# LittleWat/multichannel-semseg-with-uda

Measured on AMD Instinct MI355X. Metric: RGB-D img/s (6x480x640) MCD train step, drn_d_38, higher is better.
Workload: dtype f32 (operands split 2-way into scaled fp16, 3 cross terms on the fp16 MFMA pipe, fp32 accumulate)

## Files before the change

include/mcdseg.h:

```cpp
#ifndef MCDSEG_H
#define MCDSEG_H

#include <stddef.h>
#include <stdint.h>

#ifdef __cplusplus
extern "C" {
#endif
#pragma GCC visibility push(default)

#define MCDSEG_VERSION 101

int mcdseg_version(void);
const char* mcdseg_last_error(void);

#define MCDSEG_COMM_ID_BYTES 128
int mcdseg_comm_unique_id(void* id128);
int mcdseg_comm_init(void** comm, int32_t nranks, const void* id128, int32_t rank);
int mcdseg_comm_destroy(void* comm);
int mcdseg_allreduce(float* buf, int64_t count, void* comm, void* stream);

int32_t mcdseg_option_count(void);
const char* mcdseg_option_name(int32_t index);
int mcdseg_set_option(const char* name, int64_t value);
// ... 18 lines not shown
int mcdseg_conv_dgrad(const mcdseg_conv_desc* d, const float* dy, const float* wp_dgrad, float* dx, void* stream);
#define MCDSEG_MATH_F16X3 3
#define MCDSEG_MATH_BF16X6 6
#define MCDSEG_MATH_F16X1 1
int mcdseg_conv_split_packed_bytes(const mcdseg_conv_desc* d, int32_t math, int64_t* fprop_bytes, int64_t* dgrad_bytes);
int32_t mcdseg_conv_split_direct_ok(const mcdseg_conv_desc* d);
int64_t mcdseg_conv_split_stat_rows(const mcdseg_conv_desc* d);
int64_t mcdseg_conv_split_stat_rows_for(const mcdseg_conv_desc* d, int32_t math, int32_t presplit);
int32_t mcdseg_conv_split_window_ok(const mcdseg_conv_desc* d, int32_t math, int32_t presplit, int32_t dgrad);
int32_t mcdseg_conv_split_tile_config(int32_t M, int64_t P, int32_t presplit);
int mcdseg_absmax(const float* x, int64_t n, float* bound, void* stream);
int mcdseg_conv_split_pack_weights(const mcdseg_conv_desc* d, int32_t math, const float* w, void* wp_fprop, void* wp_dgrad,
                                   float* w_bound, void* stream);
int mcdseg_conv_split_pack_weights_multi(const int64_t* ptrs, const int32_t* dims, int32_t n, int32_t math, float* bounds,
                                         void* stream);
int mcdseg_conv_split_fprop(const mcdseg_conv_desc* d, int32_t math, const float* x, const void* x_cb, const float* x_bound,
                            const void* wp_fprop, const float* w_bound, const float* bias, float* y, float* stat_partials,
                            void* stream);
int mcdseg_conv_split_fprop_affine(const mcdseg_conv_desc* d, int32_t math, const float* x, const void* x_cb, const float* x_bound,
                                   const void* wp_fprop, const float* w_bound, const float* scale, const float* shift,
                                   const float* residual, int32_t relu, float* y, void* stream);
int mcdseg_conv_split_dgrad(const mcdseg_conv_desc* d, int32_t math, const float* dy, const void* dy_cb, const float* dy_bound,
                            const void* wp_dgrad, const float* w_bound, float* dx, void* stream);
int mcdseg_conv_split_dgrad_add(const mcdseg_conv_desc* d, int32_t math, const float* dy, const void* dy_cb, const float* dy_bound,
                                const void* wp_dgrad, const float* w_bound, const float* addend, float* dx, int32_t part, void* stream);
int64_t mcdseg_conv_split_parts(const mcdseg_conv_desc* d, int32_t math, int32_t presplit, int32_t dgrad);
int32_t mcdseg_conv_split_rest_pingpong(const mcdseg_conv_desc* d, int32_t math, int32_t presplit, int32_t dgrad);
int32_t mcdseg_conv_split_wide_pingpong(const mcdseg_conv_desc* d, int32_t math, int32_t presplit, int32_t dgrad);
int mcdseg_conv_split_fprop_part(const mcdseg_conv_desc* d, int32_t math, const float* x, const void* x_cb, const float* x_bound,
                                 const void* wp_fprop, const float* w_bound, const float* bias, float* y, float* stat_partials,
// ... 238 lines not shown
```

multichannel-semseg-with-uda_amd/csrc/conv_gemm_split.hip:

```cpp
#include <cstdlib>
#include <type_traits>

#include "conv_split_params.h"
#include "options.h"

namespace {


template <class P, int WM, int WN, int WAVES_M, int WAVES_N, bool DGRAD, bool PRESPLIT>
__global__ __launch_bounds__(256, 2) void conv_gemm_split_kernel(ConvSplitParams p) {
  constexpr int BM = 32 * WM * WAVES_M;
  constexpr int BN = 32 * WN * WAVES_N;
  constexpr int NT = 256;
  static_assert(WAVES_M * WAVES_N == 4, "4 waves per workgroup");
  constexpr int B_ITEMS = BN * 2 / NT;
  constexpr int NP = P::NP;
  constexpr int NQ = 2 * NP;
  typedef typename P::frag frag;
  constexpr int A_CHUNKS = NQ * BM;
  constexpr int A_ITERS = (A_CHUNKS + NT - 1) / NT;
  constexpr bool A_EXACT = (A_CHUNKS % NT) == 0;
  constexpr bool A_DMA = A_EXACT;
  constexpr int A_ITERS_DMA = ((2 * P::NPU * BM) % NT == 0) ? (2 * P::NPU * BM) / NT : A_ITERS;
  constexpr int A_BYTES = NQ * BM * 16, B_BYTES = NQ * BN * 16;
// ... 755 lines not shown
    for (int u = t; u < T * 2 * MT; u += 256) {
      const int mm = u % MT, r = u / MT;
      const int h = r & 1, tap = r >> 1;
      float v[8];
#pragma unroll
      for (int el = 0; el < 8; ++el) v[el] = tile[mm * row_len + (8 * h + el) * T + tap];
      typename P::frag q[NP];
      split_frag<P>(v, inv_scale, q);
      const int64_t base = ((int64_t)chunk * T + tap) * (2 * NP) * (int64_t)Mp * 8;
#pragma unroll
      for (int pc = 0; pc < NP; ++pc) *reinterpret_cast<typename P::frag*>(out + base + ((pc * 2 + h) * (int64_t)Mp + m0 + mm) * 8) = q[pc];
    }
  }
}

int split_check(const mcdseg_conv_desc* d, int math, const char* who, bool operands = true) {
  MCD_REQUIRE(d != nullptr, "%s: null descriptor", who);
  MCD_REQUIRE(mcd_math_known(math), "%s: math must be MCDSEG_MATH_BF16X6, MCDSEG_MATH_F16X3 or MCDSEG_MATH_F16X1 (got %d)", who, math);
  MCD_REQUIRE(d->N > 0 && d->Cin > 0 && d->H > 0 && d->W > 0 && d->Cout > 0, "%s: non-positive dims", who);
  MCD_REQUIRE(d->KH > 0 && d->KW > 0 && d->stride > 0 && d->dil > 0 && d->pad >= 0, "%s: bad kernel geometry", who);
  const int ho = (d->H + 2 * d->pad - d->dil * (d->KH - 1) - 1) / d->stride + 1;
  const int wo = (d->W + 2 * d->pad - d->dil * (d->KW - 1) - 1) / d->stride + 1;
  MCD_REQUIRE(ho == d->Ho && wo == d->Wo, "%s: Ho/Wo (%d,%d) do not match geometry (%d,%d)", who, d->Ho, d->Wo, ho, wo);
  MCD_REQUIRE(!operands || ((int64_t)d->N * d->Cin * d->H * d->W * 4 < (1ll << 31) && (int64_t)d->N * d->Cout * d->Ho * d->Wo * 4 < (1ll << 31)),
              "%s: activation tensor must stay below 2 GiB (32-bit buffer offsets); split the batch", who);
  return 0;
}

int64_t split_image_bytes(int math, int M, int K, int T) {
  return (int64_t)(round_up(K, 16) / 16) * T * 2 * mcd_math_pieces(math) * mcd_mp(M) * 16;
// ... 206 lines not shown
  math = mcd_storage_math(math);
  MCD_REQUIRE(ptrs && dims && n > 0 && n <= 32767, "conv_split_pack_weights_multi: bad table");
  MCD_REQUIRE(math == MCDSEG_MATH_BF16X6 || math == MCDSEG_MATH_F16X3, "conv_split_pack_weights_multi: unknown math %d", math);
  MCD_REQUIRE(math != MCDSEG_MATH_F16X3 || bounds != nullptr, "conv_split_pack_weights_multi: f16x3 needs the bounds array");
  hipStream_t st = (hipStream_t)stream;
  const unsigned pack_blocks = (unsigned)(mcd_opt(MCD_OPT_PACK_BLOCKS) > 0 ? mcd_opt(MCD_OPT_PACK_BLOCKS) : 192);
  if (math == MCDSEG_MATH_F16X3) {
    (void)hipMemsetAsync(bounds, 0, sizeof(float) * (size_t)n, st);
    hipLaunchKernelGGL(absmax_multi_kernel, dim3(48, (unsigned)n), dim3(256), 0, st, ptrs, dims);
    MCD_LAUNCH_CHECK("absmax_multi");
    hipLaunchKernelGGL(pack_weights_multi_kernel<SplitF16x3>, dim3(pack_blocks, 2u * (unsigned)n), dim3(256), 0, st, ptrs, dims);
  } else {
    hipLaunchKernelGGL(pack_weights_multi_kernel<SplitBf16x6>, dim3(pack_blocks, 2u * (unsigned)n), dim3(256), 0, st, ptrs, dims);
  }
  MCD_LAUNCH_CHECK("conv_split_pack_weights_multi");
  return 0;
}

static int split_cb_bytes(const mcdseg_conv_desc* d, int math, int C, int HW, const void* cb, int* piece_bytes, long long* piece_stride) {
  *piece_bytes = 0;
  *piece_stride = 0;
  if (cb == nullptr) return 0;
  MCD_REQUIRE((C % 8) == 0, "conv_split: a pre-split operand needs a channel count divisible by 8 (got %d)", C);
  MCD_REQUIRE(d->Ncb == 0 || d->Ncb >= d->N, "conv_split: Ncb (%d) must be 0 or at least N (%d)", d->Ncb, d->N);
  const int64_t b = (int64_t)d->N * C * HW * 2;
  MCD_REQUIRE(b < (1ll << 31), "conv_split: one piece of the pre-split operand exceeds 2 GiB; split the batch");
  *piece_bytes = (int)b;
  *piece_stride = math == MCDSEG_MATH_F16X1 ? 0 : (long long)(d->Ncb ? d->Ncb : d->N) * C * HW * 2;
  return 0;
}
// ... 218 lines not shown
```

multichannel-semseg-with-uda_amd/csrc/options.h:

```cpp
#pragma once
#include <stdint.h>

#define MCD_OPTIONS(X)                                                                                                       \
  X(BN_STATS_ONE, 1024)                     \
  X(BN_REVERSE, 1)                              \
  X(BN_V4, 1)                                         \
  X(BIGTILE_MIN_SLOTS, 1024)                               \
  X(WIDETILE_MIN_SLOTS, 1024)                                                                 \
  X(DGRAD_INTERLEAVE, 1)       \
  X(DGRAD_ADD_LDS, 1)                   \
  X(PACK_BLOCKS, 192)                               \
  X(PP_MIN_ROUNDS, 2)          \
  X(PP_CUS, 0)                 \
  X(PINGPONG, 3)               \
  X(PP_WIDE_FILL, 80)                               \
  X(PP_WIDE128, 1)                                                                                \
  X(PP_DEEP, 1)                \
  X(SKIP_DEAD_TAPS, 1)         \
  X(THIN_WINDOW, 1)                                                           \
  X(WGRAD_WGS, 1024)                                  \
  X(WGRAD_THIN_TR, 1)                                                               \
  X(WGRAD_TR64, 1)                                                    \
  X(WGRAD_BIG, 1)                                                                       \
  X(WGRAD_PP_CUS, 0)                          \
  X(WGRAD_PP, 2)                                          \
  X(WGRAD_PP3, 1)                                                                 \
// ... 13 lines not shown
```

multichannel-semseg-with-uda_amd/mcdseg/_lib.py:

```python
import ctypes
import glob
import os
import subprocess
import threading

HERE = os.path.dirname(os.path.abspath(__file__))
PKG = os.path.dirname(HERE)
REPO = os.path.dirname(PKG)
CSRC = os.path.join(PKG, "csrc")
INCLUDE = os.path.join(REPO, "include")
LIB_PATH = os.environ.get("MCDSEG_LIB") or os.path.join(HERE, "libmcdseg.so")

c_void_p, c_int, c_i32, c_i64, c_float, c_size_t = (ctypes.c_void_p, ctypes.c_int, ctypes.c_int32, ctypes.c_int64,
                                                    ctypes.c_float, ctypes.c_size_t)


class ConvDesc(ctypes.Structure):
    _fields_ = [(n, c_i32) for n in ("N", "Cin", "H", "W", "Cout", "KH", "KW", "stride", "pad", "dil", "Ho", "Wo", "Ncb")]


_P = ctypes.POINTER
_SIGNATURES = {
    "mcdseg_version": (c_int, []),
    "mcdseg_last_error": (ctypes.c_char_p, []),
# ... 26 lines not shown
    "mcdseg_up8_uncertain_loss_bwd": (c_int, [c_void_p] * 5 + [c_i64, c_void_p, c_void_p, c_float, c_void_p, c_float] + [c_void_p] * 4 +
                                      [c_i32] * 5 + [c_void_p]),
    "mcdseg_up8_std_sum": (c_int, [c_void_p] * 3 + [c_i32] * 5 + [c_void_p]),
    "mcdseg_dann_down_workspace_bytes": (c_size_t, [c_i32] * 5),
    "mcdseg_dann_down_fwd": (c_int, [c_void_p] * 6 + [c_i32] * 5 + [c_void_p]),
    "mcdseg_dann_down_bwd": (c_int, [c_void_p] * 11 + [c_i32] * 6 + [c_void_p, c_size_t, c_void_p]),
    "mcdseg_dann_tail_save_bytes": (c_size_t, [c_i32] * 2),
    "mcdseg_dann_tail_workspace_bytes": (c_size_t, [c_i32] * 2),
    "mcdseg_dann_tail_fwd": (c_int, [c_void_p] * 10 + [c_float, c_float, c_i32] + [c_void_p] * 3 + [c_i32] * 3 + [c_void_p]),
    "mcdseg_dann_tail_bwd": (c_int, [c_void_p] * 16 + [c_i32] * 4 + [c_void_p, c_size_t, c_void_p]),
    "mcdseg_depth_image_u8": (c_int, [c_void_p, c_void_p] + [c_i32] * 4 + [c_void_p]),
    "mcdseg_absmax": (c_int, [c_void_p, c_i64, c_void_p, c_void_p]),
    "mcdseg_conv_split_packed_bytes": (c_int, [_P(ConvDesc), c_i32, _P(c_i64), _P(c_i64)]),
    "mcdseg_conv_split_pack_weights": (c_int, [_P(ConvDesc), c_i32] + [c_void_p] * 5),
    "mcdseg_conv_split_pack_weights_multi": (c_int, [c_void_p, c_void_p, c_i32, c_i32, c_void_p, c_void_p]),
    "mcdseg_conv_split_fprop": (c_int, [_P(ConvDesc), c_i32] + [c_void_p] * 9),
    "mcdseg_conv_split_fprop_affine": (c_int, [_P(ConvDesc), c_i32] + [c_void_p] * 8 + [c_i32, c_void_p, c_void_p]),
    "mcdseg_conv_split_dgrad": (c_int, [_P(ConvDesc), c_i32] + [c_void_p] * 7),
    "mcdseg_conv_split_parts": (c_i64, [_P(ConvDesc), c_i32, c_i32, c_i32]),
    "mcdseg_conv_split_rest_pingpong": (c_i32, [_P(ConvDesc), c_i32, c_i32, c_i32]),
    "mcdseg_conv_split_wide_pingpong": (c_i32, [_P(ConvDesc), c_i32, c_i32, c_i32]),
    "mcdseg_conv_split_fprop_part": (c_int, [_P(ConvDesc), c_i32] + [c_void_p] * 8 + [c_i32, c_void_p]),
    "mcdseg_conv_split_dgrad_part": (c_int, [_P(ConvDesc), c_i32] + [c_void_p] * 6 + [c_i32, c_void_p]),
    "mcdseg_conv_split_dgrad_add": (c_int, [_P(ConvDesc), c_i32] + [c_void_p] * 7 + [c_i32, c_void_p]),
    "mcdseg_split_cb": (c_int, [c_void_p, c_void_p, c_void_p, c_i32, c_i32, c_i32, c_i32, c_void_p]),
    "mcdseg_split_cb_padded": (c_int, [c_void_p, c_void_p, c_void_p, c_i32, c_i32, c_i32, c_i32, c_void_p]),
    "mcdseg_unsplit_cb": (c_int, [c_void_p, c_void_p, c_i32, c_i32, c_i32, c_i32, c_void_p, c_void_p]),
    "mcdseg_stage_join": (c_int, [c_void_p] * 7 + [c_i32] * 4 + [c_void_p]),
    "mcdseg_bn_apply_cb": (c_int, [c_void_p] * 11 + [c_i32] * 5 + [c_void_p]),
    "mcdseg_bn_bwd_apply_cb": (c_int, [c_void_p] * 13 + [c_i32] * 6 + [c_void_p]),
# ... 394 lines not shown
```

multichannel-semseg-with-uda_amd/mcdseg/ops.py:

```python
import collections
import contextlib
import ctypes
import os
import threading
import types
import weakref

import torch

from . import _lib
from ._lib import ConvDesc, check, get_option, lib

WEIGHT_EPOCH = 0


def bump_weight_epoch(params=None):
    global WEIGHT_EPOCH
    if params is None:
        WEIGHT_EPOCH += 1
        return
    for p in params:
        p._mcd_epoch = getattr(p, "_mcd_epoch", 0) + 1


# ... 357 lines not shown
    members = []
    for pw in list(_PACK_REGISTRY):
        w = pw._weight() if pw._weight is not None else None
        if (w is None or pw._dims is None or pw._dims[4] != CONV_MATH or w.device != device or pw.wd is None or pw.wf is None
                or pw._dims[2] > 72):
            continue
        members.append((pw, w))
    if len(members) < 2:
        return
    members.sort(key=lambda m: m[1].data_ptr())
    sig = tuple((w.data_ptr(), pw.wf.data_ptr(), pw.wd.data_ptr()) + pw._dims for pw, w in members)
    tab = _PACK_TABLES.get((device, CONV_MATH))
    if tab is None or tab["sig"] != sig:
        n = len(members)
        bounds = torch.zeros(n, dtype=torch.float32, device=device)
        ptrs, dims = [], []
        for i, (pw, w) in enumerate(members):
            ptrs += [w.data_ptr(), pw.wf.data_ptr(), pw.wd.data_ptr(), bounds.data_ptr() + 4 * i]
            dims += [pw._dims[0], pw._dims[1], pw._dims[2], 0]
        tab = dict(sig=sig, bounds=bounds, ptrs=torch.tensor(ptrs, dtype=torch.int64).to(device),
                   dims=torch.tensor(dims, dtype=torch.int32).to(device))
        _PACK_TABLES[(device, CONV_MATH)] = tab
    if _scaled():
        for i, (pw, _) in enumerate(members):
            pw.w_bound = tab["bounds"][i:i + 1]
    n = len(members)
    nbytes = sum(4 * w.numel() + 2 * pw.wf.numel() + 2 * pw.wd.numel() for pw, w in members)
    with _timed("pack_weights_multi_kernel", (0, nbytes)):
        check(L.mcdseg_conv_split_pack_weights_multi(_p(tab["ptrs"]), _p(tab["dims"]), n, MATH_ID[CONV_MATH],
                                                     _p(tab["bounds"]) if _scaled() else None, _stream()), "conv_split_pack_weights_multi")
    for pw, w in members:
        if pw._dims[3]:
            d = ConvDesc(1, pw._dims[1], 8, 8, pw._dims[0], 7, 7, 1, 3, 1, 8, 8)
            check(L.mcdseg_conv_split_pack_weights(ctypes.byref(d), MATH_ID[CONV_MATH], _p(w.detach()), _p(pw.wf), None,
                                                   _p(pw.w_bound) if _scaled() else None, _stream()), "conv_split_pack_weights")
        pw.key = PackedWeights._key_of(w)


def _is_split(w_image):
    return w_image.dtype == torch.int16


MAX_CONV_BYTES = int(os.environ.get("MCDSEG_MAX_CONV_BYTES", str((1 << 31) - (1 << 26))))


# ... 218 lines not shown
    return _wgrad_name(d, _wgrad_variant(d, have_cb))


def _wgrad_thin_tr(desc):
    return _wgrad_variant(desc, True) == 15


def _wgrad_split_plan(desc, have_cb=False):
    return _wgrad_variant(desc, have_cb) >= 10


def _wgrad_reads_cb(desc):
    return _wgrad_variant(desc, True) >= 11 and desc.Cin % 8 == 0 and desc.Cout % 8 == 0


def _conv_wgrad(desc, x, dy, x_cb=None, dy_cb=None, x_bound=None, dy_bound=None):
    L, total = lib(), None
    if x_cb is None or dy_cb is None:
        x_cb = dy_cb = None
    pieces = _batch_pieces(desc, wgrad_cb=x_cb is not None)
    if x_cb is not None and len(pieces) > 1 and desc.Cin <= 16:
        x_cb = dy_cb = None
        pieces = _batch_pieces(desc, wgrad_cb=False)
    split = _wgrad_split_plan(desc, x_cb is not None)
    if split and x_cb is None:
        x_bound, dy_bound = _bound_or_measure(x, x_bound), _bound_or_measure(dy, dy_bound)
    for a, b, d in _launches(desc, pieces, x_cb is not None):
        ws = _ws(L.mcdseg_conv_wgrad_workspace_bytes(ctypes.byref(d)), (x if x is not None else x_cb).device)
        dw = torch.empty((desc.Cout, desc.Cin, desc.KH, desc.KW), dtype=torch.float32, device=ws.device)
        name = "" if LAUNCH_TIMER is None else (wgrad_split_kernel_name(d, x_cb is not None) if split else
                                                 wgrad_kernel_name(desc.Cout, desc.Cin, desc.KH * desc.KW))
        with _timed(name, conv_work(d)):
            if split:
                check(L.mcdseg_conv_split_wgrad(ctypes.byref(d), MATH_ID[CONV_MATH], _p(_sl(x, a, b)), _cb_slice(x_cb, a, desc.Cin, desc.H * desc.W),
                                                _p(x_bound), _p(_sl(dy, a, b)), _cb_slice(dy_cb, a, desc.Cout, desc.Ho * desc.Wo), _p(dy_bound),
                                                _p(dw), _p(ws), ctypes.c_size_t(ws.numel() * 4), _stream()), "conv_split_wgrad")
            else:
                check(L.mcdseg_conv_wgrad(ctypes.byref(d), _p(x[a:b]), _p(dy[a:b]), _p(dw), _p(ws), ctypes.c_size_t(ws.numel() * 4),
                                          _stream()), "conv_wgrad")
        _on_launch_stream(ws, dw)
        if total is None:
            total = dw
        else:
            with torch.cuda.stream(_LAUNCH.stream or torch.cuda.current_stream()):
                total.add_(dw)
    return total


OVERLAP_WGRAD = os.environ.get("MCDSEG_OVERLAP_WGRAD", "2")
if OVERLAP_WGRAD not in ("0", "1", "2"):
    raise ValueError("MCDSEG_OVERLAP_WGRAD must be 0, 1 or 2, got %r" % OVERLAP_WGRAD)
_SIDE = {}
_PENDING = {}


def _side_stream(device):
    key = device.index if device.index is not None else torch.cuda.current_device()
    if key not in _SIDE:
        _SIDE[key] = torch.cuda.Stream(device=device)
    return _SIDE[key]


def join_side_streams(device_index=None):
# ... 66 lines not shown
    if ev is not None:
        torch.cuda.current_stream().wait_event(ev)
        anchor._mcd_fwd_ev = None


def _fwd_sync_record(anchor):
    ev = torch.cuda.Event()
    ev.record(torch.cuda.current_stream())
    anchor._mcd_fwd_ev = ev


class _LateGrad(torch.autograd.Function):

    @staticmethod
    def forward(ctx, w):
        return w.view_as(w)

    @staticmethod
    def backward(ctx, g):
        join_side_streams(g.device.index)
        return g


class late_weight_grads:

    def __init__(self, root):
        self.root, self.mods = root, []

    def __enter__(self):
        if OVERLAP_WGRAD == "2" and torch.is_grad_enabled():
            for m in self.root.modules():
                if isinstance(getattr(m, "_packed", None), PackedWeights) and getattr(m, "_w_late", None) is None:
                    w = m.weight
                    if w.is_cuda and w.requires_grad and (not getattr(w, "_post_accumulate_grad_hooks", None) or
                                                          getattr(w, "_mcd_grad_sink", None) is not None):
# ... 44 lines not shown
def _conv_backward(desc, x, dy, wd, need_dx, need_dw, dy_cb=None, x_cb=None, dy_bound=None, x_bound=None, w_bound=None, defer=False, param=None,
                   dx_addend=None, dx16=False):
    mode = OVERLAP_WGRAD
    sink = getattr(param, "_mcd_grad_sink", None) if param is not None else None
    if mode == "2" and not (defer and x_cb is not None and dy_cb is not None):
        mode = "0"
    if mode != "0" and LAUNCH_TIMER is not None and LAUNCH_TIMER.wants("conv_wgrad"):
        mode = "0"
    if mode == "2" and not _room_to_defer(x.device):
        mode = "0"
        WGRAD_STREAM_STATS["no_room"] += 1
    if not (need_dx and need_dw and mode != "0"):
        if sink is not None and need_dw:
            sink(param, None)
        return ((_dgrad_any(desc, dy, wd, dy_cb, dy_bound, w_bound, dx_addend, dx16) if need_dx else None),
                (_conv_wgrad(desc, x, dy, x_cb, dy_cb, x_bound, dy_bound) if need_dw else None))
    main = torch.cuda.current_stream()
    side = _side_stream(x.device)
    key = side.device.index
    if _scaled() and dy is not None:
        dy_bound = _bound_or_measure(dy, dy_bound)
    side.wait_stream(main)
    _LAUNCH.stream, _LAUNCH.keep = side, [x, dy, x_cb, dy_cb, x_bound, dy_bound]
    try:
        dw = _conv_wgrad(desc, x, dy, x_cb, dy_cb, x_bound, dy_bound)
    finally:
        keep, _LAUNCH.stream, _LAUNCH.keep = _LAUNCH.keep, None, None
    dx = _dgrad_any(desc, dy, wd, dy_cb, dy_bound, w_bound, dx_addend, dx16)
    if mode == "1":
        main.wait_stream(side)
        if sink is not None:
            sink(param, None)
        return dx, dw
    if sink is not None:
        with torch.cuda.stream(side):
            sink(param, dw)
    WGRAD_STREAM_STATS["deferred"] += 1
    ev = torch.cuda.Event()
    ev.record(side)
    _PENDING[key] = (ev, main)
    held = _HELD.setdefault(key, collections.deque())
    held.append((ev, keep))
    while len(held) > MAX_LAG:
        main.wait_event(held.popleft()[0])
    torch.autograd.Variable._execution_engine.queue_callback(join_side_streams)
    return dx, dw


MASK_NONE = "none"
MASK_Y = "y"
MASK_Y_CB = "y_cb"
MASK_Z = "z"
MASK_BITS = "bits"


def _channel_reduce(dy, mask=MASK_NONE, src=None, z=None, mean=None, rstd=None, gamma=None, beta=None, want_bound=False, train=True):
    L = lib()
    n, c, hw = dy.shape[0], dy.shape[1], dy.shape[2] * dy.shape[3]
    ws = _ws(L.mcdseg_bn_bwd_workspace_bytes(n, c, hw), dy.device)
    dgamma = torch.empty(c, dtype=torch.float32, device=dy.device) if z is not None else None
    dbeta = torch.empty(c, dtype=torch.float32, device=dy.device)
    bound = torch.empty(1, dtype=torch.float32, device=dy.device) if want_bound else None
    tail = (int(train), n, c, hw, _p(ws), ctypes.c_size_t(ws.numel() * 4), _stream())
    if mask == MASK_BITS:
        with _timed("bn_bwd_reduce", (0, 4 * n * c * hw * 2)):
            check(L.mcdseg_bn_bwd_reduce_mask(_p(dy), _p(src), _p(z), _p(mean), _p(rstd), _p(gamma) if want_bound else None, _p(dgamma),
                                              _p(dbeta), _p(bound), *tail), "bn_bwd_reduce_mask")
    elif mask == MASK_Z:
        with _timed("bn_bwd_reduce", (0, 4 * n * c * hw * 2)):
            check(L.mcdseg_bn_bwd_reduce_zmask(_p(dy), _p(z), _p(mean), _p(rstd), _p(gamma), _p(beta), _p(dgamma), _p(dbeta), _p(bound),
                                               *tail), "bn_bwd_reduce_zmask")
    else:
        with _timed("bn_bwd_reduce", (0, 4 * n * c * hw * (1 + (mask == MASK_Y) + (z is not None)))):
            check(L.mcdseg_bn_bwd_reduce(_p(dy), _p(src) if mask == MASK_Y else None, _p(src) if mask == MASK_Y_CB else None,
                                         MATH_ID.get(CONV_MATH, 0), _p(z), _p(mean), _p(rstd), _p(dgamma), _p(dbeta),
                                         _p(gamma) if want_bound else None, _p(bound), int(train), n, c, hw, int(mask != MASK_NONE),
# ... 246 lines not shown
                                                  _p(dbeta), _p(dz_bound), mask, 1, n, c, hw, _p(ws), ctypes.c_size_t(ws.numel() * 4),
                                                  _stream()), "bn_bwd_reduce_half")
            dz_cb = torch.empty(elems, dtype=torch.int16, device=dy.device)
            if plan.has_res and need.residual:
                dres = torch.empty_like(dy) if plan.relu else dy
            p_dres = _p(dres) if plan.relu else None
            with _timed("bn_bwd_apply_half", (0, elems * (6 + (2 if mask == 4 else 0) + (2 if p_dres is not None else 0)))):
                check(L.mcdseg_bn_bwd_apply_half(_p(dy), src, _p(z), _p(ctx.z_bound), _p(mean), _p(rstd), _p(gamma), _p(beta), _p(dgamma),
                                                 _p(dbeta), _p(dz_cb), _p(dz_bound), p_dres, mask, 1, n, c, hw, _stream()),
                      "bn_bwd_apply_half")
        else:
            if plan.y_fp32:
                y, y_cb = materialize(y, y_cb, y_bound), None
            y_mask = (y if y_cb is None else None) if plan.relu else None
            src = {MASK_NONE: None, MASK_Y: y_mask, MASK_Y_CB: y_cb, MASK_BITS: ctx.rmask, MASK_Z: None if plan.use_cb else y_mask}[plan.mask]
            dgamma, dbeta, dz_bound = _channel_reduce(dy, plan.mask, src, z, mean, rstd, gamma, beta, plan.want_bound, plan.training)
            if plan.has_res and need.residual:
                dres = torch.empty_like(z) if plan.relu else dy
            if not plan.skip_dz:
                dz = torch.empty_like(z)
            dz_cb = _bn_bwd_apply(dy, plan.mask, src, plan.use_cb, z, mean, rstd, gamma, beta, dgamma, dbeta, dz, dres, dz_bound, plan.training)
            if plan.x_fp32_bwd:
                x = materialize(x, ctx.x_cb, ctx.x_bound)
            if DEBUG_TAPE is not None:
                DEBUG_TAPE.append(dict(dy=dy, dz=dz, dz_cb=dz_cb, dz_bound=dz_bound, dgamma=dgamma, dbeta=dbeta, dres=dres, shape=(n, c, hw),
                                       z=z, y=y_mask, mean=mean, rstd=rstd, gamma=gamma, beta=beta, zmask=plan.mask == MASK_Z))
            if dres is not None and plan.res_half:
                dres = pack_bf16_units(dres)
        if ctx.res_box is not None and dres is not None:
            other, last = ctx.res_box.arrive()
            if last:
                dres = dres if other is None else dres + other
            else:
                ctx.res_box.leave(dres if other is None else dres + other)
                dres = None
        addend, dx_last = ctx.in_box.arrive() if (ctx.in_box is not None and need.x) else (None, True)
        dx, dw = _conv_backward(desc, x, dz, ctx.wd, need.x, need.weight, dz_cb, x_cb, dz_bound, x_bound, ctx.w_bound, defer=ctx.defer_ok,
                                param=ctx.w_param, dx_addend=addend, dx16=ctx.x_half)
        if not dx_last:
            ctx.in_box.leave(dx)
            dx = None
        dbias = _channel_reduce(dz)[1] if (plan.has_bias and need.conv_bias) else None
        return tuple(_GroupGrads(x=dx, weight=dw, gamma=dgamma if need.gamma else None, beta=dbeta if need.beta else None, residual=dres,
                                 conv_bias=dbias))


def _conv_bn_act_inference(x, conv, bn, relu, residual):
    L = lib()
    x = _req(materialize(x), "conv input")
    residual = _req(materialize(residual) if residual is not None else None, "residual")
    desc = conv_desc(x.shape, conv.weight.shape, conv.stride[0], conv.padding[0], conv.dilation[0])
    wf, _, _ = conv._packed.get(conv.weight, desc)
    c = desc.Cout
    scale = torch.empty(c, dtype=torch.float32, device=x.device)
    shift = torch.empty(c, dtype=torch.float32, device=x.device)
    check(L.mcdseg_bn_eval_affine(_p(bn.weight), _p(bn.bias), _p(bn.running_mean), _p(bn.running_var), _p(conv.bias), c,
                                  float(bn.eps), _p(scale), _p(shift), _stream()), "bn_eval_affine")
# ... 1178 lines not shown
```

multichannel-semseg-with-uda_amd/mcdseg/optim.py:

```python
import os

import torch

from . import dist as mdist
from . import ops

_ALIGN = 64
DP_OVERLAP = os.environ.get("MCDSEG_DP_OVERLAP", "0") == "1"
DP_BUCKET_MB = float(os.environ.get("MCDSEG_DP_BUCKET_MB", "25"))


class _FlatOptimizer(torch.optim.Optimizer):
    _require_gpu = True
    _STATE = ()

    def __init__(self, params, defaults):
        super().__init__(params, defaults)
        self._flat = None

    @property
    def _name(self):
        return type(self).__name__

    def _all_params(self):
# ... 19 lines not shown
            offs.append(total)
            total += (p.numel() + _ALIGN - 1) // _ALIGN * _ALIGN
        fp = torch.zeros(total, dtype=torch.float32, device=dev)
        fs = [torch.zeros(total, dtype=torch.float32, device=dev) for _ in self._STATE]
        fg = torch.zeros(total, dtype=torch.float32, device=dev)
        views = {}
        for p, o in zip(params, offs):
            n = p.numel()
            pv = fp[o:o + n].view(p.shape)
            pv.copy_(p.data)
            p.data = pv
            sv = [f[o:o + n].view(p.shape) for f in fs]
            views[id(p)] = (o, n, sv[0], fg[o:o + n].view(p.shape)) + tuple(sv[1:])
        self._flat = dict(p=fp, g=fg, params=params, offs=offs, views=views, total=total)
        self._flat.update((key, f) for (key, _), f in zip(self._STATE, fs))
        self._adopt_state(fresh=True)
        ops.bump_weight_epoch()
        self._setup_overlap()

    def _state_views(self, p):
        t = self._flat["views"][id(p)]
        return (t[2],) + t[4:]

    def _adopt_state(self, fresh=False):
        for p in self._flat["params"]:
            st = self.state.get(p) or {}
            for (_, name), view in zip(self._STATE, self._state_views(p)):
                if st.get(name) is None:
                    if not fresh:
                        view.zero_()
# ... 110 lines not shown
        else:
            fl["views"][id(p)][3].copy_(p.grad)
            self._copied(b, p.grad)
        self._arrive(b, p)

    def _finish_overlap(self, ps):
        fl = self._flat
        self._drain(flush=True)
        buckets = {id(b): b for b in (fl["bucket_of"].get(id(p)) for p in ps) if b is not None}
        for b in buckets.values():
            if b["work"] is not None:
                b["work"].wait()
        return all(fl["bucket_of"].get(id(p)) is not None and fl["bucket_of"][id(p)]["work"] is not None and
                   not fl["bucket_of"][id(p)]["dirty"] for p in ps)

    def _reset_overlap(self):
        for b in (self._flat or {}).get("buckets", []):
            if b["work"] is not None:
                b["work"].wait()
            b["arrived"], b["work"], b["dirty"], b["ready"], b["launched"] = 0, None, False, False, False
            b["early"].clear(), b["early_seen"].clear(), b["unsunk"].clear(), b["seen"].clear(), b["events"].clear()
        if self._flat is not None and "next" in self._flat:
            self._flat["next"] = 0

    def _ensure_flat(self):
        if self._flat is None:
            self._flatten()
            return
        fl = self._flat
        for p in fl["params"]:
            o = fl["views"][id(p)][0]
# ... 22 lines not shown
                continue
            key = self._run_key(g, p)
            if cur is None or cur["key"] != key:
                cur = dict(key=key, params=[])
                runs.append(cur)
            cur["params"].append(p)
        world = mdist.world_size()
        for run in runs:
            ps = run["params"]
            o0 = fl["views"][id(ps[0])][0]
            o1, n1 = fl["views"][id(ps[-1])][0], fl["views"][id(ps[-1])][1]
            lo, hi = o0, o1 + n1
            gflat = fl["g"][lo:hi]
            reduced = bool(fl.get("buckets")) and self._finish_overlap(ps)
            if not reduced:
                gviews = [fl["views"][id(p)][3] for p in ps]
                grads = [p.grad if p.grad.dtype == torch.float32 else p.grad.float() for p in ps]
                torch._foreach_copy_(gviews, grads)
                if mdist.is_distributed():
                    mdist.all_reduce_sum_(gflat)
            self._update(fl, lo, hi, gflat, run["key"], ps, 1.0 / world)
        self._reset_overlap()
        return loss

    def zero_grad(self, set_to_none=True):
        super().zero_grad(set_to_none=set_to_none)
        if self._flat is not None:
            self._reset_overlap()

    def state_dict(self):
        sd = super().state_dict()
        sd["state"] = {k: {name: (t.clone() if torch.is_tensor(t) else t) for name, t in st.items()} for k, st in sd["state"].items()}
        return sd
# ... 69 lines not shown
```

Before: 81.65.

## Pack weights per tile in one list kernel and land grads in flat buffer

Adds a tile-list weight packing path. An absmax kernel and a pack kernel each run over a flat grid of 32x32 tiles, with each block finding its layer by binary search, instead of the fixed multi-layer launch; it is enabled by a new PACK_FORM option. Separately, weight-gradient and BN dgamma/dbeta kernels now write directly into the optimizer's flat gradient views, so the per-step foreach copy into the flat buffer is skipped for parameters that landed there. This removes a gradient copy pass and aims for better load balance in packing, at the cost of aliasing bookkeeping that must be reset each step.

```diff
diff --git a/include/mcdseg.h b/include/mcdseg.h
--- a/include/mcdseg.h
+++ b/include/mcdseg.h
@@ -56,6 +56,9 @@
                                    float* w_bound, void* stream);
 int mcdseg_conv_split_pack_weights_multi(const int64_t* ptrs, const int32_t* dims, int32_t n, int32_t math, float* bounds,
                                          void* stream);
+int32_t mcdseg_conv_split_pack_tiles(int32_t Cout, int32_t Cin, int32_t T);
+int mcdseg_conv_split_pack_weights_list(const int64_t* ptrs, const int32_t* dims, int32_t n, int32_t tiles, int32_t math,
+                                        float* bounds, void* stream);
 int mcdseg_conv_split_fprop(const mcdseg_conv_desc* d, int32_t math, const float* x, const void* x_cb, const float* x_bound,
                             const void* wp_fprop, const float* w_bound, const float* bias, float* y, float* stat_partials,
                             void* stream);
diff --git a/multichannel-semseg-with-uda_amd/csrc/conv_gemm_split.hip b/multichannel-semseg-with-uda_amd/csrc/conv_gemm_split.hip
--- a/multichannel-semseg-with-uda_amd/csrc/conv_gemm_split.hip
+++ b/multichannel-semseg-with-uda_amd/csrc/conv_gemm_split.hip
@@ -793,6 +793,153 @@
   }
 }
 
+constexpr int PACK_TILE_FLOATS = 32 * 32 * 9;
+
+__host__ __device__ inline int pack_mp(int M) { return M <= 32 ? 32 : (M <= 64 ? 64 : ((M + 127) / 128) * 128); }
+__host__ __device__ inline int pack_ct(int T) { return T <= 9 ? 32 : 16; }
+__host__ __device__ inline int pack_slices(int T) { return T <= 36 ? 1 : 2; }
+__host__ __device__ inline int pack_tiles_of(int Cout, int Cin, int T) {
+  const int ct = pack_ct(T);
+  return (pack_mp(Cout) / ct) * (pack_mp(Cin) / ct) * pack_slices(T);
+}
+
+__device__ __forceinline__ int pack_entry_of(const int32_t* __restrict__ dims, int n, int b) {
+  int lo = 0, hi = n - 1;
+  while (lo < hi) {
+    const int mid = (lo + hi + 1) >> 1;
+    if (dims[4 * mid + 3] <= b) lo = mid; else hi = mid - 1;
+  }
+  return lo;
+}
+
+__global__ __launch_bounds__(256) void absmax_list_kernel(const int64_t* __restrict__ ptrs, const int32_t* __restrict__ dims, int n,
+                                                          int total_tiles) {
+  const int b = blockIdx.x;
+  const int e = pack_entry_of(dims, n, b);
+  const int first = dims[4 * e + 3];
+  const int tiles = (e + 1 < n ? dims[4 * (e + 1) + 3] : total_tiles) - first, j = b - first;
+  if (tiles <= 0 || j >= tiles) return;
+  const float* __restrict__ x = reinterpret_cast<const float*>(ptrs[4 * e + 0]);
+  unsigned* __restrict__ out = reinterpret_cast<unsigned*>(ptrs[4 * e + 3]);
+  const int64_t cnt = (int64_t)dims[4 * e + 0] * dims[4 * e + 1] * dims[4 * e + 2];
+  int64_t head = (int64_t)((16 - (reinterpret_cast<uintptr_t>(x) & 15)) & 15) >> 2;
+  if (head > cnt) head = cnt;
+  const int64_t n4 = (cnt - head) >> 2;
+  const uint4* __restrict__ x4 = reinterpret_cast<const uint4*>(x + head);
+  const int64_t q0 = n4 * j / tiles, q1 = n4 * (j + 1) / tiles;
+  auto amax4 = [](uint4 q) {
+    const unsigned a = q.x & 0x7FFFFFFFu, b2 = q.y & 0x7FFFFFFFu, c = q.z & 0x7FFFFFFFu, d = q.w & 0x7FFFFFFFu;
+    const unsigned ab = a > b2 ? a : b2, cd = c > d ? c : d;
+    return ab > cd ? ab : cd;
+  };
+  unsigned m = 0u;
+  int64_t i = q0 + threadIdx.x;
+  for (; i + 768 < q1; i += 1024) {
+    const uint4 v0 = x4[i], v1 = x4[i + 256], v2 = x4[i + 512], v3 = x4[i + 768];
+    const unsigned a = amax4(v0), b2 = amax4(v1), c = amax4(v2), d = amax4(v3);
+    const unsigned ab = a > b2 ? a : b2, cd = c > d ? c : d, t = ab > cd ? ab : cd;
+    m = t > m ? t : m;
+  }
+  for (; i < q1; i += 256) {
+    const unsigned t = amax4(x4[i]);
+    m = t > m ? t : m;
+  }
+  if (j == 0) {
+    const int64_t tail0 = head + (n4 << 2);
+    for (int64_t k = threadIdx.x; k < head + (cnt - tail0); k += 256) {
+      const unsigned t = __float_as_uint(x[k < head ? k : tail0 + (k - head)]) & 0x7FFFFFFFu;
+      m = t > m ? t : m;
+    }
+  }
+  for (int o = 1; o < 64; o <<= 1) {
+    const unsigned t = __shfl_xor(m, o);
+    m = t > m ? t : m;
+  }
+  __shared__ unsigned wave_max[4];
+  if ((threadIdx.x & 63) == 0) wave_max[threadIdx.x >> 6] = m;
+  __syncthreads();
+  if (threadIdx.x == 0) {
+    const unsigned a = wave_max[0] > wave_max[1] ? wave_max[0] : wave_max[1], c = wave_max[2] > wave_max[3] ? wave_max[2] : wave_max[3];
+    m = a > c ? a : c;
+    if (m > __atomic_load_n(out, __ATOMIC_RELAXED)) atomicMax(out, m);
+  }
+}
+
+template <class P>
+__global__ __launch_bounds__(256) void pack_weights_list_kernel(const int64_t* __restrict__ ptrs, const int32_t* __restrict__ dims, int n) {
+  constexpr int NP = P::NP;
+  __shared__ float tile[PACK_TILE_FLOATS + 32];
+  const int b = blockIdx.x;
+  const int e = pack_entry_of(dims, n, b);
+  const float* __restrict__ w = reinterpret_cast<const float*>(ptrs[4 * e + 0]);
+  typename P::elem* __restrict__ out_f = reinterpret_cast<typename P::elem*>(ptrs[4 * e + 1]);
+  typename P::elem* __restrict__ out_d = reinterpret_cast<typename P::elem*>(ptrs[4 * e + 2]);
+  const float inv_scale = 1.f / operand_scale<P>(reinterpret_cast<const float*>(ptrs[4 * e + 3]));
+  const int Cout = dims[4 * e + 0], Cin = dims[4 * e + 1], T = dims[4 * e + 2];
+  const int CT = pack_ct(T), slices = pack_slices(T);
+  const int Mpf = pack_mp(Cout), Mpd = pack_mp(Cin);
+  const int Kpf = ((Cin + 15) / 16) * 16, Kpd = ((Cout + 15) / 16) * 16;
+  int tl = b - dims[4 * e + 3];
+  if (T > 72 || tl >= pack_tiles_of(Cout, Cin, T)) return;
+  const int s = tl % slices;
+  tl /= slices;
+  const int ci_tiles = Mpd / CT;
+  const int co0 = (tl / ci_tiles) * CT, ci0 = (tl % ci_tiles) * CT;
+  const int t0 = s * 36, TT = slices == 1 ? T : (T - t0 < 36 ? T - t0 : 36);
+  const int cols = CT * TT, row_len = cols + 1;
+  const int t = threadIdx.x, lane = t & 63, wave = t >> 6;
+  for (int r = wave; r < CT; r += 4) {
+    const bool row_ok = co0 + r < Cout;
+    const float* __restrict__ src = w + ((int64_t)(co0 + r) * Cin + ci0) * T;
+    float* __restrict__ dst = tile + r * row_len;
+    if (slices == 1) {
+      const int ok_cols = row_ok ? (Cin - ci0 < CT ? (Cin - ci0 > 0 ? (Cin - ci0) * T : 0) : cols) : 0;
+      for (int c = lane; c < cols; c += 256) {
+        const int c1 = c + 64, c2 = c + 128, c3 = c + 192;
+        const float v0 = c < ok_cols ? src[c] : 0.f, v1 = c1 < ok_cols ? src[c1] : 0.f;
+        const float v2 = c2 < ok_cols ? src[c2] : 0.f, v3 = c3 < ok_cols ? src[c3] : 0.f;
+        dst[c] = v0;
+        if (c1 < cols) dst[c1] = v1;
+        if (c2 < cols) dst[c2] = v2;
+        if (c3 < cols) dst[c3] = v3;
+      }
+    } else {
+      for (int c = lane; c < cols; c += 64) {
+        const int ci = c / TT, tap = c - ci * TT;
+        dst[c] = (row_ok && ci0 + ci < Cin) ? src[ci * T + t0 + tap] : 0.f;
+      }
+    }
+  }
+  __syncthreads();
+  const int per_img = (CT / 16) * TT * 2 * CT;
+  for (int u = t; u < 2 * per_img; u += 256) {
+    const int mode = u >= per_img;
+    int r = mode ? u - per_img : u;
+    const int mm = r & (CT - 1);
+    r >>= CT == 32 ? 5 : 4;
+    const int h = r & 1;
+    r >>= 1;
+    const int tap = r % TT, ch = r / TT;
+    typename P::elem* __restrict__ out = mode ? out_d : out_f;
+    const int k0 = (mode ? co0 : ci0) + 16 * ch;
+    if (out == nullptr || k0 >= (mode ? Kpd : Kpf)) continue;
+    float v[8];
+    if (mode == 0) {
+#pragma unroll
+      for (int el = 0; el < 8; ++el) v[el] = tile[mm * row_len + (16 * ch + 8 * h + el) * TT + tap];
+    } else {
+#pragma unroll
+      for (int el = 0; el < 8; ++el) v[el] = tile[(16 * ch + 8 * h + el) * row_len + mm * TT + tap];
+    }
+    typename P::frag q[NP];
+    split_frag<P>(v, inv_scale, q);
+    const int Mp = mode ? Mpd : Mpf, m = (mode ? ci0 : co0) + mm;
+    const int64_t base = ((int64_t)(k0 / 16) * T + t0 + tap) * (2 * NP) * (int64_t)Mp * 8;
+#pragma unroll
+    for (int pc = 0; pc < NP; ++pc) *reinterpret_cast<typename P::frag*>(out + base + ((pc * 2 + h) * (int64_t)Mp + m) * 8) = q[pc];
+  }
+}
+
 int split_check(const mcdseg_conv_desc* d, int math, const char* who, bool operands = true) {
   MCD_REQUIRE(d != nullptr, "%s: null descriptor", who);
   MCD_REQUIRE(mcd_math_known(math), "%s: math must be MCDSEG_MATH_BF16X6, MCDSEG_MATH_F16X3 or MCDSEG_MATH_F16X1 (got %d)", who, math);
@@ -1029,6 +1176,31 @@
     hipLaunchKernelGGL(pack_weights_multi_kernel<SplitBf16x6>, dim3(pack_blocks, 2u * (unsigned)n), dim3(256), 0, st, ptrs, dims);
   }
   MCD_LAUNCH_CHECK("conv_split_pack_weights_multi");
+  return 0;
+}
+
+extern "C" int32_t mcdseg_conv_split_pack_tiles(int32_t Cout, int32_t Cin, int32_t T) {
+  if (Cout <= 0 || Cin <= 0 || T <= 0 || T > 72) return 0;
+  return pack_tiles_of(Cout, Cin, T);
+}
+
+extern "C" int mcdseg_conv_split_pack_weights_list(const int64_t* ptrs, const int32_t* dims, int32_t n, int32_t tiles, int32_t math,
+                                                   float* bounds, void* stream) {
+  if (mcd_opt(MCD_OPT_PACK_FORM) == 0) return mcdseg_conv_split_pack_weights_multi(ptrs, dims, n, math, bounds, stream);
+  math = mcd_storage_math(math);
+  MCD_REQUIRE(ptrs && dims && n > 0 && n <= 32767 && tiles >= n, "conv_split_pack_weights_list: bad table");
+  MCD_REQUIRE(math == MCDSEG_MATH_BF16X6 || math == MCDSEG_MATH_F16X3, "conv_split_pack_weights_list: unknown math %d", math);
+  MCD_REQUIRE(math != MCDSEG_MATH_F16X3 || bounds != nullptr, "conv_split_pack_weights_list: f16x3 needs the bounds array");
+  hipStream_t st = (hipStream_t)stream;
+  if (math == MCDSEG_MATH_F16X3) {
+    (void)hipMemsetAsync(bounds, 0, sizeof(float) * (size_t)n, st);
+    hipLaunchKernelGGL(absmax_list_kernel, dim3((unsigned)tiles), dim3(256), 0, st, ptrs, dims, n, tiles);
+    MCD_LAUNCH_CHECK("absmax_list");
+    hipLaunchKernelGGL(pack_weights_list_kernel<SplitF16x3>, dim3((unsigned)tiles), dim3(256), 0, st, ptrs, dims, n);
+  } else {
+    hipLaunchKernelGGL(pack_weights_list_kernel<SplitBf16x6>, dim3((unsigned)tiles), dim3(256), 0, st, ptrs, dims, n);
+  }
+  MCD_LAUNCH_CHECK("conv_split_pack_weights_list");
   return 0;
 }
 
diff --git a/multichannel-semseg-with-uda_amd/csrc/options.h b/multichannel-semseg-with-uda_amd/csrc/options.h
--- a/multichannel-semseg-with-uda_amd/csrc/options.h
+++ b/multichannel-semseg-with-uda_amd/csrc/options.h
@@ -10,6 +10,7 @@
   X(DGRAD_INTERLEAVE, 1)       \
   X(DGRAD_ADD_LDS, 1)                   \
   X(PACK_BLOCKS, 192)                               \
+  X(PACK_FORM, 1)              \
   X(PP_MIN_ROUNDS, 2)          \
   X(PP_CUS, 0)                 \
   X(PINGPONG, 3)               \
diff --git a/multichannel-semseg-with-uda_amd/mcdseg/_lib.py b/multichannel-semseg-with-uda_amd/mcdseg/_lib.py
--- a/multichannel-semseg-with-uda_amd/mcdseg/_lib.py
+++ b/multichannel-semseg-with-uda_amd/mcdseg/_lib.py
@@ -64,6 +64,8 @@
     "mcdseg_conv_split_packed_bytes": (c_int, [_P(ConvDesc), c_i32, _P(c_i64), _P(c_i64)]),
     "mcdseg_conv_split_pack_weights": (c_int, [_P(ConvDesc), c_i32] + [c_void_p] * 5),
     "mcdseg_conv_split_pack_weights_multi": (c_int, [c_void_p, c_void_p, c_i32, c_i32, c_void_p, c_void_p]),
+    "mcdseg_conv_split_pack_tiles": (c_i32, [c_i32] * 3),
+    "mcdseg_conv_split_pack_weights_list": (c_int, [c_void_p, c_void_p, c_i32, c_i32, c_i32, c_void_p, c_void_p]),
     "mcdseg_conv_split_fprop": (c_int, [_P(ConvDesc), c_i32] + [c_void_p] * 9),
     "mcdseg_conv_split_fprop_affine": (c_int, [_P(ConvDesc), c_i32] + [c_void_p] * 8 + [c_i32, c_void_p, c_void_p]),
     "mcdseg_conv_split_dgrad": (c_int, [_P(ConvDesc), c_i32] + [c_void_p] * 7),
diff --git a/multichannel-semseg-with-uda_amd/mcdseg/ops.py b/multichannel-semseg-with-uda_amd/mcdseg/ops.py
--- a/multichannel-semseg-with-uda_amd/mcdseg/ops.py
+++ b/multichannel-semseg-with-uda_amd/mcdseg/ops.py
@@ -395,11 +395,12 @@
     if tab is None or tab["sig"] != sig:
         n = len(members)
         bounds = torch.zeros(n, dtype=torch.float32, device=device)
-        ptrs, dims = [], []
+        ptrs, dims, tiles = [], [], 0
         for i, (pw, w) in enumerate(members):
             ptrs += [w.data_ptr(), pw.wf.data_ptr(), pw.wd.data_ptr(), bounds.data_ptr() + 4 * i]
-            dims += [pw._dims[0], pw._dims[1], pw._dims[2], 0]
-        tab = dict(sig=sig, bounds=bounds, ptrs=torch.tensor(ptrs, dtype=torch.int64).to(device),
+            dims += [pw._dims[0], pw._dims[1], pw._dims[2], tiles]
+            tiles += L.mcdseg_conv_split_pack_tiles(*pw._dims[:3])
+        tab = dict(sig=sig, bounds=bounds, tiles=tiles, ptrs=torch.tensor(ptrs, dtype=torch.int64).to(device),
                    dims=torch.tensor(dims, dtype=torch.int32).to(device))
         _PACK_TABLES[(device, CONV_MATH)] = tab
     if _scaled():
@@ -408,8 +409,8 @@
     n = len(members)
     nbytes = sum(4 * w.numel() + 2 * pw.wf.numel() + 2 * pw.wd.numel() for pw, w in members)
     with _timed("pack_weights_multi_kernel", (0, nbytes)):
-        check(L.mcdseg_conv_split_pack_weights_multi(_p(tab["ptrs"]), _p(tab["dims"]), n, MATH_ID[CONV_MATH],
-                                                     _p(tab["bounds"]) if _scaled() else None, _stream()), "conv_split_pack_weights_multi")
+        check(L.mcdseg_conv_split_pack_weights_list(_p(tab["ptrs"]), _p(tab["dims"]), n, tab["tiles"], MATH_ID[CONV_MATH],
+                                                    _p(tab["bounds"]) if _scaled() else None, _stream()), "conv_split_pack_weights_list")
     for pw, w in members:
         if pw._dims[3]:
             d = ConvDesc(1, pw._dims[1], 8, 8, pw._dims[0], 7, 7, 1, 3, 1, 8, 8)
@@ -658,7 +659,7 @@
     return _wgrad_variant(desc, True) >= 11 and desc.Cin % 8 == 0 and desc.Cout % 8 == 0
 
 
-def _conv_wgrad(desc, x, dy, x_cb=None, dy_cb=None, x_bound=None, dy_bound=None):
+def _conv_wgrad(desc, x, dy, x_cb=None, dy_cb=None, x_bound=None, dy_bound=None, out=None):
     L, total = lib(), None
     if x_cb is None or dy_cb is None:
         x_cb = dy_cb = None
@@ -671,7 +672,8 @@
         x_bound, dy_bound = _bound_or_measure(x, x_bound), _bound_or_measure(dy, dy_bound)
     for a, b, d in _launches(desc, pieces, x_cb is not None):
         ws = _ws(L.mcdseg_conv_wgrad_workspace_bytes(ctypes.byref(d)), (x if x is not None else x_cb).device)
-        dw = torch.empty((desc.Cout, desc.Cin, desc.KH, desc.KW), dtype=torch.float32, device=ws.device)
+        dw = out if (out is not None and total is None) else torch.empty((desc.Cout, desc.Cin, desc.KH, desc.KW), dtype=torch.float32,
+                                                                          device=ws.device)
         name = "" if LAUNCH_TIMER is None else (wgrad_split_kernel_name(d, x_cb is not None) if split else
                                                  wgrad_kernel_name(desc.Cout, desc.Cin, desc.KH * desc.KW))
         with _timed(name, conv_work(d)):
@@ -691,6 +693,20 @@
     return total
 
 
+GRAD_LANDING = os.environ.get("MCDSEG_GRAD_LANDING", "1") != "0"
+GRAD_LANDING_STATS = {"landed": 0}
+
+
+def grad_slot(param):
+    rec = getattr(param, "_mcd_grad_slot", None) if param is not None else None
+    if (rec is None or rec[1] or not GRAD_LANDING or (LAUNCH_TIMER is not None and LAUNCH_TIMER.wants("conv_wgrad")) or param.grad is not None
+            or getattr(param, "_mcd_grad_sink", None) is not None or getattr(param, "_post_accumulate_grad_hooks", None)):
+        return None
+    rec[1] = True
+    GRAD_LANDING_STATS["landed"] += 1
+    return rec[0]
+
+
 OVERLAP_WGRAD = os.environ.get("MCDSEG_OVERLAP_WGRAD", "2")
 if OVERLAP_WGRAD not in ("0", "1", "2"):
     raise ValueError("MCDSEG_OVERLAP_WGRAD must be 0, 1 or 2, got %r" % OVERLAP_WGRAD)
@@ -787,11 +803,14 @@
 
     @staticmethod
     def forward(ctx, w):
+        ctx.slot = getattr(w, "_mcd_grad_slot", None)
         return w.view_as(w)
 
     @staticmethod
     def backward(ctx, g):
         join_side_streams(g.device.index)
+        if ctx.slot is not None and g.data_ptr() == ctx.slot[0].data_ptr():
+            return g.detach()
         return g
 
 
@@ -866,7 +885,7 @@
         if sink is not None and need_dw:
             sink(param, None)
         return ((_dgrad_any(desc, dy, wd, dy_cb, dy_bound, w_bound, dx_addend, dx16) if need_dx else None),
-                (_conv_wgrad(desc, x, dy, x_cb, dy_cb, x_bound, dy_bound) if need_dw else None))
+                (_conv_wgrad(desc, x, dy, x_cb, dy_cb, x_bound, dy_bound, out=grad_slot(param)) if need_dw else None))
     main = torch.cuda.current_stream()
     side = _side_stream(x.device)
     key = side.device.index
@@ -875,7 +894,7 @@
     side.wait_stream(main)
     _LAUNCH.stream, _LAUNCH.keep = side, [x, dy, x_cb, dy_cb, x_bound, dy_bound]
     try:
-        dw = _conv_wgrad(desc, x, dy, x_cb, dy_cb, x_bound, dy_bound)
+        dw = _conv_wgrad(desc, x, dy, x_cb, dy_cb, x_bound, dy_bound, out=grad_slot(param))
     finally:
         keep, _LAUNCH.stream, _LAUNCH.keep = _LAUNCH.keep, None, None
     dx = _dgrad_any(desc, dy, wd, dy_cb, dy_bound, w_bound, dx_addend, dx16)
@@ -906,12 +925,13 @@
 MASK_BITS = "bits"
 
 
-def _channel_reduce(dy, mask=MASK_NONE, src=None, z=None, mean=None, rstd=None, gamma=None, beta=None, want_bound=False, train=True):
+def _channel_reduce(dy, mask=MASK_NONE, src=None, z=None, mean=None, rstd=None, gamma=None, beta=None, want_bound=False, train=True,
+                    out=(None, None)):
     L = lib()
     n, c, hw = dy.shape[0], dy.shape[1], dy.shape[2] * dy.shape[3]
     ws = _ws(L.mcdseg_bn_bwd_workspace_bytes(n, c, hw), dy.device)
-    dgamma = torch.empty(c, dtype=torch.float32, device=dy.device) if z is not None else None
-    dbeta = torch.empty(c, dtype=torch.float32, device=dy.device)
+    dgamma = (out[0] if out[0] is not None else torch.empty(c, dtype=torch.float32, device=dy.device)) if z is not None else None
+    dbeta = out[1] if out[1] is not None else torch.empty(c, dtype=torch.float32, device=dy.device)
     bound = torch.empty(1, dtype=torch.float32, device=dy.device) if want_bound else None
     tail = (int(train), n, c, hw, _p(ws), ctypes.c_size_t(ws.numel() * 4), _stream())
     if mask == MASK_BITS:
@@ -1188,7 +1208,8 @@
                 y, y_cb = materialize(y, y_cb, y_bound), None
             y_mask = (y if y_cb is None else None) if plan.relu else None
             src = {MASK_NONE: None, MASK_Y: y_mask, MASK_Y_CB: y_cb, MASK_BITS: ctx.rmask, MASK_Z: None if plan.use_cb else y_mask}[plan.mask]
-            dgamma, dbeta, dz_bound = _channel_reduce(dy, plan.mask, src, z, mean, rstd, gamma, beta, plan.want_bound, plan.training)
+            slots = (grad_slot(gamma) if need.gamma else None, grad_slot(beta) if need.beta else None)
+            dgamma, dbeta, dz_bound = _channel_reduce(dy, plan.mask, src, z, mean, rstd, gamma, beta, plan.want_bound, plan.training, slots)
             if plan.has_res and need.residual:
                 dres = torch.empty_like(z) if plan.relu else dy
             if not plan.skip_dz:
@@ -1215,6 +1236,9 @@
             ctx.in_box.leave(dx)
             dx = None
         dbias = _channel_reduce(dz)[1] if (plan.has_bias and need.conv_bias) else None
+        if not plan.half:
+            dgamma = dgamma.detach() if slots[0] is not None else dgamma
+            dbeta = dbeta.detach() if slots[1] is not None else dbeta
         return tuple(_GroupGrads(x=dx, weight=dw, gamma=dgamma if need.gamma else None, beta=dbeta if need.beta else None, residual=dres,
                                  conv_bias=dbias))
 
diff --git a/multichannel-semseg-with-uda_amd/mcdseg/optim.py b/multichannel-semseg-with-uda_amd/mcdseg/optim.py
--- a/multichannel-semseg-with-uda_amd/mcdseg/optim.py
+++ b/multichannel-semseg-with-uda_amd/mcdseg/optim.py
@@ -57,6 +57,8 @@
             views[id(p)] = (o, n, sv[0], fg[o:o + n].view(p.shape)) + tuple(sv[1:])
         self._flat = dict(p=fp, g=fg, params=params, offs=offs, views=views, total=total)
         self._flat.update((key, f) for (key, _), f in zip(self._STATE, fs))
+        for p in params:
+            p._mcd_grad_slot = [views[id(p)][3], False]
         self._adopt_state(fresh=True)
         ops.bump_weight_epoch()
         self._setup_overlap()
@@ -197,7 +199,16 @@
         return all(fl["bucket_of"].get(id(p)) is not None and fl["bucket_of"][id(p)]["work"] is not None and
                    not fl["bucket_of"][id(p)]["dirty"] for p in ps)
 
+    @staticmethod
+    def _landed(fl, p):
+        g, v = p.grad, fl["views"][id(p)][3]
+        return g.data_ptr() == v.data_ptr() and g.dtype == v.dtype and g.shape == v.shape and g.is_contiguous()
+
     def _reset_overlap(self):
+        for p in (self._flat or {}).get("params", []):
+            rec = getattr(p, "_mcd_grad_slot", None)
+            if rec is not None:
+                rec[1] = False
         for b in (self._flat or {}).get("buckets", []):
             if b["work"] is not None:
                 b["work"].wait()
@@ -250,9 +261,11 @@
             gflat = fl["g"][lo:hi]
             reduced = bool(fl.get("buckets")) and self._finish_overlap(ps)
             if not reduced:
-                gviews = [fl["views"][id(p)][3] for p in ps]
-                grads = [p.grad if p.grad.dtype == torch.float32 else p.grad.float() for p in ps]
-                torch._foreach_copy_(gviews, grads)
+                rest = [p for p in ps if not self._landed(fl, p)]
+                if rest:
+                    gviews = [fl["views"][id(p)][3] for p in rest]
+                    grads = [p.grad if p.grad.dtype == torch.float32 else p.grad.float() for p in rest]
+                    torch._foreach_copy_(gviews, grads)
                 if mdist.is_distributed():
                     mdist.all_reduce_sum_(gflat)
             self._update(fl, lo, hi, gflat, run["key"], ps, 1.0 / world)
```

Result: no change. 81.95, median of 6 (+0.4%).
